# RainbowZL0/swin-unet-image-fusion

Measured on AMD Instinct MI355X. Metric: fused image-pairs/sec at 256x256, win=8, higher is better.
Workload: dtype bf16; 1 GPU; B=16/GPU 256x256 IR/visible pairs, win=8, 5-level Swin-UNet fusion forward (BASELINE configs[1]); global_batch=16, precision_mode=fast, residual_stream=fp32, hip_graph=True, steps_in_flight=3, kernel_schedule=throughput, collective=none, weights=random-init (numpy PCG64 recipe, seed 0)

## Files before the change

### swin_unet_image_fusion_amd/csrc/kernels_win96.hip

```cpp
#include "win_host.h"

#include <cstdlib>

namespace swf {
namespace {

using namespace wf;

template <int HID_>
struct G96 {
    static constexpr int C = 96, HID = HID_, HEADS = 8, D = 12, TC = 3, VT = 4, KS = 6;
    static constexpr int NT1 = HID / 32, KU = HID / 16;
    static_assert(HID % 32 == 0, "hidden tiles");
    static constexpr int F_QKV = 0;
    static constexpr int F_P = 144;
    static constexpr int F_W1 = 192;
    static constexpr int F_W2 = F_W1 + 12 * NT1;
    static constexpr int NFRAG = F_W2 + 6 * KU;
    static constexpr int V_LN1G = 0, V_LN1B = 48, V_LN2G = 96, V_LN2B = 144, V_B2 = 192, V_BQ = 240, V_BK = 304, V_B1 = 368;
    static constexpr int VHF = V_B1 + 16 * NT1, VSTREAM = 2 * VHF + 128;
    static constexpr size_t p_vec = size_t(NFRAG) * 1024;
    static constexpr size_t p_bias = (p_vec + size_t(VSTREAM) * 4 + 15) / 16 * 16;
    static constexpr size_t p_total = p_bias + size_t(2) * 2 * 16 * 64 * 4;
    static constexpr size_t l_k = 0, l_v = 32 * 1024, l_vec = 64 * 1024, l_total = l_vec + size_t(2) * VSTREAM * 4;
    static constexpr size_t l_vec8 = 96 * 1024, l_total8 = l_vec8 + size_t(2) * VSTREAM * 4;
    static constexpr size_t p_total16 = p_bias + size_t(15) * 16 * 64 * 4;
    static constexpr size_t l_k16 = 0, l_v16 = 64 * 1024, l_vec16 = 128 * 1024, l_total16 = l_vec16 + size_t(2) * VSTREAM * 4;
    static_assert(l_total16 <= 160 * 1024, "LDS");
};


__device__ __forceinline__ void layernorm96(const f32x16 (&x)[3], const float* vec, int goff, int boff, u32x4 (&xh)[6], u32x4 (&xl)[6]) {
    float s = 0.f;
#pragma unroll
    for (int T = 0; T < 3; ++T)
#pragma unroll
        for (int i = 0; i < 16; ++i) s += x[T][i];
    const float mean = sum_halves(s) * (1.0f / 96.0f);
    float q = 0.f;
#pragma unroll
    for (int T = 0; T < 3; ++T)
#pragma unroll
        for (int i = 0; i < 16; ++i) {
            const float d = x[T][i] - mean;
            q += d * d;
        }
    const float rstd = __builtin_amdgcn_rsqf(sum_halves(q) * (1.0f / 96.0f) + 1e-5f);
#pragma unroll
    for (int T = 0; T < 3; ++T) {
        float n[16];
#pragma unroll
        for (int a = 0; a < 4; ++a) {
            const float4 g = *reinterpret_cast<const float4*>(vec + goff + 16 * T + 4 * a);
            const float4 b = *reinterpret_cast<const float4*>(vec + boff + 16 * T + 4 * a);
            n[4 * a + 0] = (x[T][4 * a + 0] - mean) * rstd * g.x + b.x;
            n[4 * a + 1] = (x[T][4 * a + 1] - mean) * rstd * g.y + b.y;
            n[4 * a + 2] = (x[T][4 * a + 2] - mean) * rstd * g.z + b.z;
            n[4 * a + 3] = (x[T][4 * a + 3] - mean) * rstd * g.w + b.w;
        }
        split8(n, xh[2 * T], xl[2 * T]);
        split8(n + 8, xh[2 * T + 1], xl[2 * T + 1]);
    }
}

__device__ __forceinline__ void raw96(const f32x16 (&x)[3], u32x4 (&xh)[6], u32x4 (&xl)[6]) {
#pragma unroll
    for (int T = 0; T < 3; ++T) {
        float n[16];
#pragma unroll
        for (int i = 0; i < 16; ++i) n[i] = x[T][i];
        split8(n, xh[2 * T], xl[2 * T]);
        split8(n + 8, xh[2 * T + 1], xl[2 * T + 1]);
    }
}

template <int NH = 8>
__device__ __forceinline__ void attention96(const u32x4* ksrc, const u32x4* vsrc, const u32x4 (&qf)[NH / 2][2], const f32x16 (&bias)[2],
                                            bool half1, f32x16 (&o)[NH / 2]) {
    const f32x16 zero16 = {0.f, 0.f, 0.f, 0.f, 0.f, 0.f, 0.f, 0.f, 0.f, 0.f, 0.f, 0.f, 0.f, 0.f, 0.f, 0.f};
#pragma unroll
    for (int T = 0; T < NH / 2; ++T) o[T] = zero16;
#pragma unroll
    for (int h = 0; h < NH; ++h) {
        const int T = h >> 1, sp = h & 1;
        const u32x4 ka0 = ksrc[((0 * 4 + T) * 2 + sp) * 64], ka1 = ksrc[((1 * 4 + T) * 2 + sp) * 64];
        u32x4 qm = qf[T][sp];
        float mx;
        {
            f32x16 s0 = mfma_f16(ka0, qm, bias[0]);
            mx = max3f(s0[0], s0[1], s0[2]);
#pragma unroll
            for (int i = 3; i < 15; i += 2) mx = max3f(mx, s0[i], s0[i + 1]);
            mx = __builtin_fmaxf(mx, s0[15]);
        }
        {
            f32x16 s1 = mfma_f16(ka1, qm, bias[1]);
#pragma unroll
            for (int i = 0; i < 16; i += 2) mx = max3f(mx, s1[i], s1[i + 1]);
        }
        mx = max_halves(mx);
        {
            const f16 nm = (f16)(-mx);
            qm[2] |= half1 ? ((unsigned)__builtin_bit_cast(unsigned short, nm) << 16) : 0u;
        }
        f32x16 t;
#pragma unroll
        for (int kt = 0; kt < 2; ++kt) {
            f32x16 sc = mfma_f16(kt ? ka1 : ka0, qm, bias[kt]);
#pragma unroll
            for (int s2 = 0; s2 < 2; ++s2) {
                float p[8];
#pragma unroll
                for (int j = 0; j < 8; ++j) p[j] = __builtin_amdgcn_exp2f(sc[8 * s2 + j]);
                const u32x4 pf = pack8_f16(p);
                const u32x4 va = vsrc[(T * 4 + 2 * kt + s2) * 64];
                t = mfma_f16(va, pf, (kt == 0 && s2 == 0) ? zero16 : t);
                __builtin_amdgcn_sched_barrier(0);
            }
        }
#pragma unroll
        for (int j = 0; j < 8; ++j) o[T][8 * sp + j] = t[8 * sp + j];
        __builtin_amdgcn_sched_barrier(0);
    }
}

template <int HID, int WS, int MODE = WIN_BLOCK, bool RAW = false>
__global__ __launch_bounds__(256, 2) void window96_kernel(WinArgs args) {
    using G = G96<HID>;
    static_assert(WS == 7 || WS == 8, "window side");
    static_assert(!RAW || MODE != WIN_BLOCK, "RAW belongs to the half-block modes");
    constexpr bool ATT = MODE != WIN_MLP, MLP = MODE != WIN_ATTN;
    extern __shared__ __attribute__((aligned(16))) char smem96[];
    u32x4* kimg = reinterpret_cast<u32x4*>(smem96 + G::l_k);
    u32x4* vimg = reinterpret_cast<u32x4*>(smem96 + G::l_v);
    float* lvec = reinterpret_cast<float*>(smem96 + G::l_vec);

    const int tid = threadIdx.x, lane = tid & 63, wave = tid >> 6;
    const int ws = wave >> 1, qb = wave & 1, r = lane & 31, hf = lane >> 5;
    const int H = args.H, W = args.W, nwx = ATT ? W / WS : 1, nwy = ATT ? H / WS : 1, npi = nwx * nwy;
    const int nwin = ATT ? args.B * npi : (max(args.ntok[0], args.ntok[1]) + 63) / 64;
    const int sh = args.shift ? WS / 2 : 0;
    const int kvs = args.cross ? 1 - ws : ws;

    const __amdgpu_buffer_rsrc_t wrs = __builtin_amdgcn_make_buffer_rsrc(const_cast<char*>(uniform_ptr(args.packed[ws])), 0, (int)G::p_total, 0x00020000);
    const __amdgpu_buffer_rsrc_t krs = __builtin_amdgcn_make_buffer_rsrc(const_cast<char*>(uniform_ptr(args.packed[kvs])), 0, (int)G::p_total, 0x00020000);
    const int act_bytes = ATT ? args.B * H * W * 96 * 4 : args.ntok[ws] * 96 * 4;
    const __amdgpu_buffer_rsrc_t irs = __builtin_amdgcn_make_buffer_rsrc(const_cast<float*>(uniform_ptr(args.in[ws])), 0, act_bytes, 0x00020000);
    const __amdgpu_buffer_rsrc_t ors = __builtin_amdgcn_make_buffer_rsrc(uniform_ptr(args.out[ws]), 0, (MODE == WIN_BLOCK || args.out[ws]) ? act_bytes : 0, 0x00020000);
    const unsigned loff = (unsigned)lane * 16u;
    auto WF = [&](int f) { return __builtin_bit_cast(u32x4, __builtin_amdgcn_raw_buffer_load_b128(wrs, loff, f * 1024, 0)); };
    auto WK = [&](int f) { return __builtin_bit_cast(u32x4, __builtin_amdgcn_raw_buffer_load_b128(krs, loff, f * 1024, 0)); };
    const float* vec = lvec + ws * G::VSTREAM + hf * G::VHF;
    const float* veck = lvec + kvs * G::VSTREAM + hf * G::VHF;
    const float* vecv = lvec + kvs * G::VSTREAM + 2 * G::VHF;
    const bool half1 = hf != 0;
    const bool col_masked = half1 != (((r >> 2) & 1) != 0);
    const f32x16 zero16 = {0.f, 0.f, 0.f, 0.f, 0.f, 0.f, 0.f, 0.f, 0.f, 0.f, 0.f, 0.f, 0.f, 0.f, 0.f, 0.f};

    for (int win = blockIdx.x; win < nwin; win += gridDim.x) {
        SWF_WF_FENCE();
        const int b = win / npi, wrem = win - b * npi;
        const int wy = wrem / nwx, wx = wrem - wy * nwx;
        const int ty = 4 * qb + (r >> 3), tx = r & 7;
        int oy = wy * WS + ty + sh, ox = wx * WS + tx + sh;
        oy = oy >= H ? oy - H : oy;
        ox = ox >= W ? ox - W : ox;
        const unsigned tokoff = [&]() -> unsigned {
            if constexpr (ATT) {
                return (WS == 8 || (ty < WS && tx < WS)) ? (unsigned)((((b * H + oy) * W + ox) * 96 + 4 * hf) * 4) : 0x80000000u;
            } else {
                const int tok = 64 * win + 32 * qb + r;
                return tok < args.ntok[ws] ? (unsigned)((tok * 96 + 4 * hf) * 4) : 0x80000000u;
            }
        }();
        auto load_rows = [&](f32x16 (&x)[3]) {
#pragma unroll
            for (int a = 0; a < 12; ++a) {
                const f32x4 v = __builtin_bit_cast(f32x4, __builtin_amdgcn_raw_buffer_load_b128(irs, tokoff, 32 * a, 0));
                x[a >> 2][4 * (a & 3)] = v.x; x[a >> 2][4 * (a & 3) + 1] = v.y; x[a >> 2][4 * (a & 3) + 2] = v.z; x[a >> 2][4 * (a & 3) + 3] = v.w;
            }
        };

        f32x16 res[3];
        if constexpr (ATT) {
        u32x4 qf[4][2];
        {
            u32x4 wq[2][6];
            auto req = [&](int hp, u32x4 (&dst)[6]) {
                const int m = hp >> 3, f0 = G::F_QKV + ((hp >> 1) * 6 + 3 * (hp & 1)) * 2;
#pragma unroll
                for (int i = 0; i < 6; ++i) dst[i] = m == 0 ? WF(f0 + i) : WK(f0 + i);
            };
            req(0, wq[0]);
            u32x4 xh[6], xl[6];
            {
                f32x16 x[3];
                load_rows(x);
                if (win == (int)blockIdx.x) {
                    static_assert(G::VSTREAM % 4 == 0 && G::p_vec % 16 == 0, "vector sections move as 16-byte groups");
                    fill_vectors<G::VSTREAM / 4, 256>(lvec, args.packed[0] + G::p_vec, args.packed[1] + G::p_vec, tid);
                    __syncthreads();
                }
                if constexpr (RAW) raw96(x, xh, xl);
                else layernorm96(x, vec, G::V_LN1G, G::V_LN1B, xh, xl);
            }
            f32x16 acc = zero16;
#pragma unroll
            for (int hp = 0; hp < 24; ++hp) {
                const int m = hp >> 3, T = (hp >> 1) & 3, half = hp & 1;
                SWF_WF_FENCE();
                if (hp + 1 < 24) req(hp + 1, wq[(hp + 1) & 1]);
                SWF_WF_FENCE();
                const u32x4 (&w)[6] = wq[hp & 1];
                const bool skip = RAW && (m == 0 ? ws == 1 : ws == 0);
                if (skip && hp == 9 && win != (int)blockIdx.x) __syncthreads();
                if (half == 0) acc = zero16;
                if (!skip) {
#pragma unroll
                for (int s = 0; s < 3; ++s) {
                    const int ks = 3 * half + s;
                    acc = m < 2 ? mma3(w[2 * s], w[2 * s + 1], xh[ks], xl[ks], acc)
                                : mma3(xh[ks], xl[ks], w[2 * s], w[2 * s + 1], acc);
                }
                }
                if (half == 1 && !skip) {
                    float t[16];
                    if (m < 2) {
                        const float* bsrc = m == 0 ? vec + G::V_BQ : veck + G::V_BK;
#pragma unroll
                        for (int g = 0; g < 4; ++g) {
                            const float4 bb = *reinterpret_cast<const float4*>(bsrc + 16 * T + 4 * g);
                            t[4 * g] = acc[4 * g] + bb.x; t[4 * g + 1] = acc[4 * g + 1] + bb.y; t[4 * g + 2] = acc[4 * g + 2] + bb.z; t[4 * g + 3] = acc[4 * g + 3] + bb.w;
                        }
                        if (m == 0) {
                            qf[T][0] = pack8_f16(t);
                            qf[T][1] = pack8_f16(t + 8);
                        } else {
                            if (T == 0 && win != (int)blockIdx.x) __syncthreads();
                            u32x4* kdst = kimg + (((kvs * 2 + qb) * 4 + T) * 2) * 64 + lane;
                            kdst[0] = pack8_f16(t);
                            kdst[64] = pack8_f16(t + 8);
                        }
                    } else {
                        const float bv = vecv[32 * T + r];
#pragma unroll
                        for (int i = 0; i < 16; ++i) t[i] = acc[i] + bv;
                        u32x4* vdst = vimg + ((kvs * 4 + T) * 4 + 2 * qb) * 64 + lane;
                        vdst[0] = pack8_f16(t);
                        vdst[64] = pack8_f16(t + 8);
                    }
                }
            }
        }
        f32x16 bias[2];
        load_bias_tiles(wrs, loff, (int)G::p_bias, __builtin_amdgcn_readfirstlane(qb) * 2, bias);
        __syncthreads();
        if (RAW && ws == 1) continue;

        f32x16 o[4];
        {
            const bool rowv = args.shift && wy == nwy - 1, colv = args.shift && wx == nwx - 1;
            const u32x4* ksrc = kimg + (ws * 16) * 64 + lane;
            const u32x4* vsrc = vimg + (ws * 16) * 64 + lane;
            if (rowv || colv) {
                const float pen0 = ((rowv && qb == 1) || (colv && col_masked)) ? -INFINITY : 0.f;
                const float pen1 = ((rowv && qb == 0) || (colv && col_masked)) ? -INFINITY : 0.f;
#pragma unroll
                for (int i = 0; i < 16; ++i) { bias[0][i] += pen0; bias[1][i] += pen1; }
            }
            attention96(ksrc, vsrc, qf, bias, half1, o);
        }

        u32x4 wp[2][6];
        auto reqp = [&](int ks, u32x4 (&dst)[6]) {
#pragma unroll
            for (int To = 0; To < 3; ++To) { dst[2 * To] = WF(G::F_P + (To * 8 + ks) * 2); dst[2 * To + 1] = WF(G::F_P + (To * 8 + ks) * 2 + 1); }
        };
        SWF_WF_FENCE();
        if constexpr (RAW) { res[0] = zero16; res[1] = zero16; res[2] = zero16; }
        else load_rows(res);
        reqp(0, wp[0]);
        SWF_WF_FENCE();
        {
            u32x4 oh[8], ol[8];
#pragma unroll
            for (int h = 0; h < 8; ++h) {
                const int T = h >> 1, sp = h & 1;
                float lo_, den;
                halves(o[T][8 * sp + 4], lo_, den);
                const float inv = __builtin_amdgcn_rcpf(den);
                float t[8];
#pragma unroll
                for (int j = 0; j < 8; ++j) t[j] = o[T][8 * sp + j] * inv;
                split8(t, oh[h], ol[h]);
            }
#pragma unroll
            for (int ks = 0; ks < 8; ++ks) {
                SWF_WF_FENCE();
                if (ks + 1 < 8) reqp(ks + 1, wp[(ks + 1) & 1]);
                SWF_WF_FENCE();
                const u32x4 (&w)[6] = wp[ks & 1];
#pragma unroll
                for (int To = 0; To < 3; ++To) res[To] = mma3(w[2 * To], w[2 * To + 1], oh[ks], ol[ks], res[To]);
            }
        }

        } else {
            load_rows(res);
            if (win == (int)blockIdx.x) {
                fill_vectors<G::VSTREAM / 4, 256>(lvec, args.packed[0] + G::p_vec, args.packed[1] + G::p_vec, tid);
                __syncthreads();
            }
        }

        if constexpr (MLP) {
            u32x4 w1[12];
            auto req1 = [&](int tI) {
#pragma unroll
                for (int i = 0; i < 12; ++i) w1[i] = WF(G::F_W1 + tI * 12 + i);
            };
            req1(0);
            SWF_WF_FENCE();
            u32x4 xh[6], xl[6];
            if constexpr (RAW) { raw96(res, xh, xl); res[0] = zero16; res[1] = zero16; res[2] = zero16; }
            else layernorm96(res, vec, G::V_LN2G, G::V_LN2B, xh, xl);
#pragma unroll 1
            for (int tI = 0; tI < G::NT1; ++tI) {
                SWF_WF_FENCE();
                u32x4 w2[3][2][2];
#pragma unroll
                for (int To = 0; To < 3; ++To)
#pragma unroll
                    for (int s2 = 0; s2 < 2; ++s2) {
                        w2[To][s2][0] = WF(G::F_W2 + (To * G::KU + 2 * tI + s2) * 2);
                        w2[To][s2][1] = WF(G::F_W2 + (To * G::KU + 2 * tI + s2) * 2 + 1);
                    }
                SWF_WF_FENCE();
                f32x16 acc = zero16;
#pragma unroll
                for (int s = 0; s < 6; ++s) acc = mma3(w1[2 * s], w1[2 * s + 1], xh[s], xl[s], acc);
                SWF_WF_FENCE();
                if (tI + 1 < G::NT1) req1(tI + 1);
                SWF_WF_FENCE();
                float e[16];
                elu_tile(acc, vec + G::V_B1 + 16 * tI, e);
#pragma unroll
                for (int s2 = 0; s2 < 2; ++s2) {
                    u32x4 hh, hl;
                    split8(e + 8 * s2, hh, hl);
#pragma unroll
                    for (int To = 0; To < 3; ++To) res[To] = mma3(w2[To][s2][0], w2[To][s2][1], hh, hl, res[To]);
                }
            }
#pragma unroll
            for (int a = 0; a < 12; ++a) {
                const float4 b2 = *reinterpret_cast<const float4*>(vec + G::V_B2 + 4 * a);
                res[a >> 2][4 * (a & 3)] += b2.x; res[a >> 2][4 * (a & 3) + 1] += b2.y; res[a >> 2][4 * (a & 3) + 2] += b2.z; res[a >> 2][4 * (a & 3) + 3] += b2.w;
            }
        }

#pragma unroll
        for (int a = 0; a < 12; ++a) {
            const f32x4 v = {res[a >> 2][4 * (a & 3)], res[a >> 2][4 * (a & 3) + 1], res[a >> 2][4 * (a & 3) + 2], res[a >> 2][4 * (a & 3) + 3]};
            __builtin_amdgcn_raw_buffer_store_b128(__builtin_bit_cast(u32x4, v), ors, tokoff, 32 * a, 0);
        }
    }

    if (args.warm[0]) warm_next_block<256>(args, tid);
}


#ifdef W96_PROBE
__device__ unsigned long long w96_probe[16];
#define W96_STAMP(i) do { if (blockIdx.x == 0 && threadIdx.x == 0) w96_probe[i] = wall_clock64(); } while (0)
#else
#define W96_STAMP(i) do { } while (0)
#endif

template <int HID, int WS>
__global__ __launch_bounds__(512) void window96x8_kernel(WinArgs args) {
    using G = G96<HID>;
    static_assert(WS == 7 || WS == 8, "window side");
    static_assert(G::NT1 % 2 == 0, "hidden tiles split over the two feature halves");
    constexpr int NTH = G::NT1 / 2;
    extern __shared__ __attribute__((aligned(16))) char smem96[];
    u32x4* kimg = reinterpret_cast<u32x4*>(smem96 + G::l_k);
    u32x4* vimg = reinterpret_cast<u32x4*>(smem96 + G::l_v);
    f32x4* xch = reinterpret_cast<f32x4*>(smem96);
    float* lvec = reinterpret_cast<float*>(smem96 + G::l_vec8);

    const int tid = threadIdx.x, lane = tid & 63, wave = __builtin_amdgcn_readfirstlane(tid >> 6);
    const int ws = wave >> 2, qb = (wave >> 1) & 1, fh = wave & 1, r = lane & 31, hf = lane >> 5;
    const int H = args.H, W = args.W, nwx = W / WS, nwy = H / WS, npi = nwx * nwy;
    const int nwin = args.B * npi;
    const int sh = args.shift ? WS / 2 : 0;
    const int kvs = args.cross ? 1 - ws : ws;

    const __amdgpu_buffer_rsrc_t wrs = __builtin_amdgcn_make_buffer_rsrc(const_cast<char*>(uniform_ptr(args.packed[ws])), 0, (int)G::p_total, 0x00020000);
    const __amdgpu_buffer_rsrc_t krs = __builtin_amdgcn_make_buffer_rsrc(const_cast<char*>(uniform_ptr(args.packed[kvs])), 0, (int)G::p_total, 0x00020000);
    const int act_bytes = args.B * H * W * 96 * 4;
    const __amdgpu_buffer_rsrc_t irs = __builtin_amdgcn_make_buffer_rsrc(const_cast<float*>(uniform_ptr(args.in[ws])), 0, act_bytes, 0x00020000);
    const __amdgpu_buffer_rsrc_t ors = __builtin_amdgcn_make_buffer_rsrc(uniform_ptr(args.out[ws]), 0, act_bytes, 0x00020000);
    const unsigned loff = (unsigned)lane * 16u;
    auto WF = [&](int f) { return __builtin_bit_cast(u32x4, __builtin_amdgcn_raw_buffer_load_b128(wrs, loff, f * 1024, 0)); };
    auto WK = [&](int f) { return __builtin_bit_cast(u32x4, __builtin_amdgcn_raw_buffer_load_b128(krs, loff, f * 1024, 0)); };
    const float* vec = lvec + ws * G::VSTREAM + hf * G::VHF;
    const float* veck = lvec + kvs * G::VSTREAM + hf * G::VHF;
    const float* vecv = lvec + kvs * G::VSTREAM + 2 * G::VHF;
    const bool half1 = hf != 0;
    const bool col_masked = half1 != (((r >> 2) & 1) != 0);
    const f32x16 zero16 = {0.f, 0.f, 0.f, 0.f, 0.f, 0.f, 0.f, 0.f, 0.f, 0.f, 0.f, 0.f, 0.f, 0.f, 0.f, 0.f};
    auto put = [&](const f32x16 (&p)[3]) {
#pragma unroll
        for (int a = 0; a < 12; ++a)
            xch[(wave * 12 + a) * 64 + lane] = f32x4{p[a >> 2][4 * (a & 3)], p[a >> 2][4 * (a & 3) + 1], p[a >> 2][4 * (a & 3) + 2], p[a >> 2][4 * (a & 3) + 3]};
    };
    auto add_partner = [&](f32x16 (&p)[3]) {
#pragma unroll
        for (int a = 0; a < 12; ++a) {
            const f32x4 o = xch[((wave ^ 1) * 12 + a) * 64 + lane];
            p[a >> 2][4 * (a & 3)] += o[0]; p[a >> 2][4 * (a & 3) + 1] += o[1]; p[a >> 2][4 * (a & 3) + 2] += o[2]; p[a >> 2][4 * (a & 3) + 3] += o[3];
        }
    };

    W96_STAMP(0);
    for (int win = blockIdx.x; win < nwin; win += gridDim.x) {
        W96_STAMP(11 + (win != (int)blockIdx.x));
        SWF_WF_FENCE();
        const int b = win / npi, wrem = win - b * npi;
        const int wy = wrem / nwx, wx = wrem - wy * nwx;
        const int ty = 4 * qb + (r >> 3), tx = r & 7;
        int oy = wy * WS + ty + sh, ox = wx * WS + tx + sh;
        oy = oy >= H ? oy - H : oy;
        ox = ox >= W ? ox - W : ox;
        const unsigned tokoff = (WS == 8 || (ty < WS && tx < WS)) ? (unsigned)((((b * H + oy) * W + ox) * 96 + 4 * hf) * 4) : 0x80000000u;
        auto load_rows = [&](f32x16 (&x)[3]) {
#pragma unroll
            for (int a = 0; a < 12; ++a) {
                const f32x4 v = __builtin_bit_cast(f32x4, __builtin_amdgcn_raw_buffer_load_b128(irs, tokoff, 32 * a, 0));
                x[a >> 2][4 * (a & 3)] = v.x; x[a >> 2][4 * (a & 3) + 1] = v.y; x[a >> 2][4 * (a & 3) + 2] = v.z; x[a >> 2][4 * (a & 3) + 3] = v.w;
            }
        };

        u32x4 qf[2][2];
        {
            constexpr int PD = 4;
            u32x4 wq[PD][6];
            auto req = [&](int hp, u32x4 (&dst)[6]) {
                const int m = hp >> 2, f0 = G::F_QKV + ((m * 4 + ((hp >> 1) & 1)) * 6 + 3 * (hp & 1)) * 2 + fh * 24;
#pragma unroll
                for (int i = 0; i < 6; ++i) dst[i] = m == 0 ? WF(f0 + i) : WK(f0 + i);
            };
            req(0, wq[0]);
            u32x4 xh[6], xl[6];
            {
                f32x16 x[3];
                load_rows(x);
#pragma unroll
                for (int p = 1; p < PD - 1; ++p) req(p, wq[p]);
                if (win == (int)blockIdx.x) {
                    static_assert(G::VSTREAM % 4 == 0 && G::p_vec % 16 == 0, "vector sections move as 16-byte groups");
                    fill_vectors<G::VSTREAM / 4, 512>(lvec, args.packed[0] + G::p_vec, args.packed[1] + G::p_vec, tid);
                    __syncthreads();
                }
                layernorm96(x, vec, G::V_LN1G, G::V_LN1B, xh, xl);
            }
            W96_STAMP(1);
            f32x16 acc = zero16;
#pragma unroll
            for (int hp = 0; hp < 12; ++hp) {
                const int m = hp >> 2, Tl = (hp >> 1) & 1, half = hp & 1, T = 2 * fh + Tl;
                SWF_WF_FENCE();
                if (hp + PD - 1 < 12) req(hp + PD - 1, wq[(hp + PD - 1) % PD]);
                SWF_WF_FENCE();
                const u32x4 (&w)[6] = wq[hp % PD];
                if (half == 0) acc = zero16;
#pragma unroll
                for (int s = 0; s < 3; ++s) {
                    const int ks = 3 * half + s;
                    acc = m < 2 ? mma3(w[2 * s], w[2 * s + 1], xh[ks], xl[ks], acc)
                                : mma3(xh[ks], xl[ks], w[2 * s], w[2 * s + 1], acc);
                }
                if (half == 1) {
                    float t[16];
                    if (m < 2) {
                        const float* bsrc = m == 0 ? vec + G::V_BQ : veck + G::V_BK;
#pragma unroll
                        for (int g = 0; g < 4; ++g) {
                            const float4 bb = *reinterpret_cast<const float4*>(bsrc + 16 * T + 4 * g);
                            t[4 * g] = acc[4 * g] + bb.x; t[4 * g + 1] = acc[4 * g + 1] + bb.y; t[4 * g + 2] = acc[4 * g + 2] + bb.z; t[4 * g + 3] = acc[4 * g + 3] + bb.w;
                        }
                        if (m == 0) {
                            qf[Tl][0] = pack8_f16(t);
                            qf[Tl][1] = pack8_f16(t + 8);
                        } else {
                            if (Tl == 0 && win != (int)blockIdx.x) __syncthreads();
                            u32x4* kdst = kimg + (((kvs * 2 + qb) * 4 + T) * 2) * 64 + lane;
                            kdst[0] = pack8_f16(t);
                            kdst[64] = pack8_f16(t + 8);
                        }
                    } else {
                        const float bv = vecv[32 * T + r];
#pragma unroll
                        for (int i = 0; i < 16; ++i) t[i] = acc[i] + bv;
                        u32x4* vdst = vimg + ((kvs * 4 + T) * 4 + 2 * qb) * 64 + lane;
                        vdst[0] = pack8_f16(t);
                        vdst[64] = pack8_f16(t + 8);
                    }
                }
            }
        }
        W96_STAMP(2);
        f32x16 bias[2];
#pragma unroll
        for (int kt = 0; kt < 2; ++kt)
#pragma unroll
            for (int a = 0; a < 4; ++a) {
                const f32x4 v = __builtin_bit_cast(f32x4, __builtin_amdgcn_raw_buffer_load_b128(wrs, loff, (int)G::p_bias + ((qb * 2 + kt) * 4 + a) * 1024, 0));
                bias[kt][4 * a] = v.x; bias[kt][4 * a + 1] = v.y; bias[kt][4 * a + 2] = v.z; bias[kt][4 * a + 3] = v.w;
            }
        __syncthreads();
        W96_STAMP(3);

        f32x16 o[2];
        {
            const bool rowv = args.shift && wy == nwy - 1, colv = args.shift && wx == nwx - 1;
            const u32x4* ksrc = kimg + (ws * 16 + fh * 4) * 64 + lane;
            const u32x4* vsrc = vimg + (ws * 16 + fh * 8) * 64 + lane;
            if (rowv || colv) {
                const float pen0 = ((rowv && qb == 1) || (colv && col_masked)) ? -INFINITY : 0.f;
                const float pen1 = ((rowv && qb == 0) || (colv && col_masked)) ? -INFINITY : 0.f;
#pragma unroll
                for (int i = 0; i < 16; ++i) { bias[0][i] += pen0; bias[1][i] += pen1; }
            }
            attention96<4>(ksrc, vsrc, qf, bias, half1, o);
        }
        W96_STAMP(4);

        f32x16 res[3];
        {
            u32x4 wp[4][6];
#pragma unroll
            for (int ks = 0; ks < 4; ++ks)
#pragma unroll
                for (int To = 0; To < 3; ++To) {
                    wp[ks][2 * To] = WF(G::F_P + (To * 8 + ks) * 2 + fh * 8);
                    wp[ks][2 * To + 1] = WF(G::F_P + (To * 8 + ks) * 2 + 1 + fh * 8);
                }
            SWF_WF_FENCE();
            if (fh == 0) load_rows(res);
            else { res[0] = zero16; res[1] = zero16; res[2] = zero16; }
            SWF_WF_FENCE();
            u32x4 oh[4], ol[4];
#pragma unroll
            for (int h = 0; h < 4; ++h) {
                const int T = h >> 1, sp = h & 1;
                float lo_, den;
                halves(o[T][8 * sp + 4], lo_, den);
                const float inv = __builtin_amdgcn_rcpf(den);
                float t[8];
#pragma unroll
                for (int j = 0; j < 8; ++j) t[j] = o[T][8 * sp + j] * inv;
                split8(t, oh[h], ol[h]);
            }
#pragma unroll
            for (int ks = 0; ks < 4; ++ks)
#pragma unroll
                for (int To = 0; To < 3; ++To) res[To] = mma3(wp[ks][2 * To], wp[ks][2 * To + 1], oh[ks], ol[ks], res[To]);
        }
        W96_STAMP(5);
        __syncthreads();
        put(res);
        __syncthreads();
        add_partner(res);
        W96_STAMP(6);

        {
            u32x4 w1[12], w2[3][2][2];
            auto f1 = [&](int tI, int i) { return WF(G::F_W1 + tI * 12 + i + fh * (NTH * 12)); };
            auto f2 = [&](int tI, int To, int s2, int hl) { return WF(G::F_W2 + (To * G::KU + 2 * tI + s2) * 2 + hl + fh * (NTH * 4)); };
#pragma unroll
            for (int i = 0; i < 12; ++i) w1[i] = f1(0, i);
            SWF_WF_FENCE();
            u32x4 xh[6], xl[6];
            layernorm96(res, vec, G::V_LN2G, G::V_LN2B, xh, xl);
            if (fh != 0) { res[0] = zero16; res[1] = zero16; res[2] = zero16; }
            W96_STAMP(7);
#pragma unroll
            for (int s2 = 0; s2 < 2; ++s2)
#pragma unroll
                for (int To = 0; To < 3; ++To) { w2[To][s2][0] = f2(0, To, s2, 0); w2[To][s2][1] = f2(0, To, s2, 1); }
            SWF_WF_FENCE();
#pragma unroll 1
            for (int tI = 0; tI < NTH; ++tI) {
                const int tn = tI + 1 < NTH ? tI + 1 : tI;
                f32x16 acc = zero16;
#pragma unroll
                for (int s = 0; s < 6; ++s) {
                    acc = mma3(w1[2 * s], w1[2 * s + 1], xh[s], xl[s], acc);
                    SWF_WF_FENCE();
                    w1[2 * s] = f1(tn, 2 * s); w1[2 * s + 1] = f1(tn, 2 * s + 1);
                    SWF_WF_FENCE();
                }
                float e[16];
#pragma unroll
                for (int g = 0; g < 4; ++g) {
                    const float4 b1 = *reinterpret_cast<const float4*>(vec + G::V_B1 + 16 * (fh * NTH + tI) + 4 * g);
                    const float bb[4] = {b1.x, b1.y, b1.z, b1.w};
#pragma unroll
                    for (int j = 0; j < 4; ++j) {
                        const float u = acc[4 * g + j] + bb[j];
                        const float L = __builtin_fmaf(__builtin_amdgcn_exp2f(u), kLog2e, -kLog2e);
                        e[4 * g + j] = __builtin_amdgcn_fmed3f(u, L, 0.f);
                    }
                }
#pragma unroll
                for (int s2 = 0; s2 < 2; ++s2) {
                    u32x4 hh, hl;
                    split8(e + 8 * s2, hh, hl);
#pragma unroll
                    for (int To = 0; To < 3; ++To) {
                        res[To] = mma3(w2[To][s2][0], w2[To][s2][1], hh, hl, res[To]);
                        SWF_WF_FENCE();
                        w2[To][s2][0] = f2(tn, To, s2, 0); w2[To][s2][1] = f2(tn, To, s2, 1);
                        SWF_WF_FENCE();
                    }
                }
            }
        }
        W96_STAMP(8);
        __syncthreads();
        put(res);
        __syncthreads();
        add_partner(res);
#pragma unroll
        for (int a = 0; a < 12; ++a) {
            const float4 b2 = *reinterpret_cast<const float4*>(vec + G::V_B2 + 4 * a);
            res[a >> 2][4 * (a & 3)] += b2.x; res[a >> 2][4 * (a & 3) + 1] += b2.y; res[a >> 2][4 * (a & 3) + 2] += b2.z; res[a >> 2][4 * (a & 3) + 3] += b2.w;
        }

        W96_STAMP(9);
#pragma unroll
        for (int a = 0; a < 12; ++a) {
            if ((a >= 6) != (fh != 0)) continue;
            const f32x4 v = {res[a >> 2][4 * (a & 3)], res[a >> 2][4 * (a & 3) + 1], res[a >> 2][4 * (a & 3) + 2], res[a >> 2][4 * (a & 3) + 3]};
            __builtin_amdgcn_raw_buffer_store_b128(__builtin_bit_cast(u32x4, v), ors, tokoff, 32 * a, 0);
        }
    }

    W96_STAMP(10);
    if (args.warm[0]) {
        const int nsl = max(1, (int)gridDim.x / 8), sl = ((int)blockIdx.x / 8) % nsl;
        const int lines = (args.warm_bytes + 127) / 128;
        const int per = (lines + nsl - 1) / nsl, l0 = sl * per, l1 = min(lines, l0 + per);
        unsigned acc = 0;
        for (int s2 = 0; s2 < 2; ++s2)
            for (int l = l0 + tid; l < l1; l += 512) acc ^= *reinterpret_cast<const unsigned*>(args.warm[s2] + (size_t)l * 128);
        if (acc == 0x9e3779b9u && args.B < 0) args.out[0][0] = 0.f;
    }
}


template <int HID>
__global__ __launch_bounds__(256, 1) void window96w16_kernel(WinArgs args) {
    using G = G96<HID>;
    extern __shared__ __attribute__((aligned(16))) char smem96w[];
    u32x4* kimg = reinterpret_cast<u32x4*>(smem96w + G::l_k16);
    u32x4* vimg = reinterpret_cast<u32x4*>(smem96w + G::l_v16);
    float* lvec = reinterpret_cast<float*>(smem96w + G::l_vec16);

    const int tid = threadIdx.x, lane = tid & 63, wave = tid >> 6;
    const int ws = blockIdx.y, r = lane & 31, hf = lane >> 5;
    const int H = args.H, W = args.W, nwx = W / 16, nwy = H / 16, npi = nwx * nwy;
    const int nwin = args.B * npi;
    const int sh = args.shift ? 8 : 0;
    const int src = args.cross ? 1 - ws : ws;

    static_assert(G::VSTREAM % 4 == 0 && G::p_vec % 16 == 0, "vector sections move as 16-byte groups");
                    fill_vectors<G::VSTREAM / 4, 256>(lvec, args.packed[0] + G::p_vec, args.packed[1] + G::p_vec, tid);
    const __amdgpu_buffer_rsrc_t wrs = __builtin_amdgcn_make_buffer_rsrc(const_cast<char*>(args.packed[ws]), 0, (int)G::p_total16, 0x00020000);
    const int act_bytes = args.B * H * W * 96 * 4;
    const __amdgpu_buffer_rsrc_t irs = __builtin_amdgcn_make_buffer_rsrc(const_cast<float*>(args.in[ws]), 0, act_bytes, 0x00020000);
    const __amdgpu_buffer_rsrc_t srs = __builtin_amdgcn_make_buffer_rsrc(const_cast<float*>(args.in[src]), 0, act_bytes, 0x00020000);
    const __amdgpu_buffer_rsrc_t ors = __builtin_amdgcn_make_buffer_rsrc(args.out[ws], 0, act_bytes, 0x00020000);
    const unsigned loff = (unsigned)lane * 16u;
    auto WF = [&](int f) { return __builtin_bit_cast(u32x4, __builtin_amdgcn_raw_buffer_load_b128(wrs, loff, f * 1024, 0)); };
    const float* vec = lvec + ws * G::VSTREAM + hf * G::VHF;
    const float* vecs = lvec + src * G::VSTREAM + hf * G::VHF;
    const float* vecv = lvec + ws * G::VSTREAM + 2 * G::VHF;
    const bool half1 = hf != 0;
    const f32x16 zero16 = {0.f, 0.f, 0.f, 0.f, 0.f, 0.f, 0.f, 0.f, 0.f, 0.f, 0.f, 0.f, 0.f, 0.f, 0.f, 0.f};
    __syncthreads();

    for (int win = blockIdx.x; win < nwin; win += gridDim.x) {
        SWF_WF_FENCE();
        const int b = win / npi, wrem = win - b * npi;
        const int wy = wrem / nwx, wx = wrem - wy * nwx;
        auto tokoff_of = [&](int j) {
            int oy = wy * 16 + 2 * j + (r >> 4) + sh, ox = wx * 16 + (r & 15) + sh;
            oy = oy >= H ? oy - H : oy;
            ox = ox >= W ? ox - W : ox;
            return (unsigned)((((b * H + oy) * W + ox) * 96 + 4 * hf) * 4);
        };
        auto load_rows = [&](const __amdgpu_buffer_rsrc_t& rs, unsigned tokoff, f32x16 (&x)[3]) {
#pragma unroll
            for (int a = 0; a < 12; ++a) {
                const f32x4 v = __builtin_bit_cast(f32x4, __builtin_amdgcn_raw_buffer_load_b128(rs, tokoff, 32 * a, 0));
                x[a >> 2][4 * (a & 3)] = v.x; x[a >> 2][4 * (a & 3) + 1] = v.y; x[a >> 2][4 * (a & 3) + 2] = v.z; x[a >> 2][4 * (a & 3) + 3] = v.w;
            }
        };

        u32x4 qf[2][4][2];
#pragma unroll
        for (int jj = 0; jj < 2; ++jj)
#pragma unroll
            for (int T = 0; T < 4; ++T) { qf[jj][T][0] = u32x4{0u, 0u, 0u, 0u}; qf[jj][T][1] = u32x4{0u, 0u, 0u, 0u}; }
#pragma unroll 1
        for (int jj = 0; jj < 2; ++jj) {
            const int j = 2 * wave + jj;
            const unsigned tokoff = tokoff_of(j);
            u32x4 wq[2][6];
            auto req = [&](int hp, u32x4 (&dst)[6]) {
                const int f0 = G::F_QKV + ((hp >> 1) * 6 + 3 * (hp & 1)) * 2;
#pragma unroll
                for (int i = 0; i < 6; ++i) dst[i] = WF(f0 + i);
            };
            req(0, wq[0]);
            u32x4 xh[6], xl[6], kh[6], kl[6];
            {
                f32x16 x[3];
                load_rows(irs, tokoff, x);
                layernorm96(x, vec, G::V_LN1G, G::V_LN1B, xh, xl);
                if (args.cross) {
                    load_rows(srs, tokoff, x);
                    layernorm96(x, vecs, G::V_LN1G, G::V_LN1B, kh, kl);
                } else {
#pragma unroll
                    for (int s2 = 0; s2 < 6; ++s2) { kh[s2] = xh[s2]; kl[s2] = xl[s2]; }
                }
            }
#pragma unroll
            for (int T = 0; T < 4; ++T) { qf[0][T][0] = qf[1][T][0]; qf[0][T][1] = qf[1][T][1]; }
            f32x16 acc = zero16;
#pragma unroll
            for (int hp = 0; hp < 24; ++hp) {
                const int m = hp >> 3, T = (hp >> 1) & 3, half = hp & 1;
                SWF_WF_FENCE();
                if (hp + 1 < 24) req(hp + 1, wq[(hp + 1) & 1]);
                SWF_WF_FENCE();
                const u32x4 (&w)[6] = wq[hp & 1];
                if (half == 0) acc = zero16;
#pragma unroll
                for (int s2 = 0; s2 < 3; ++s2) {
                    const int ks = 3 * half + s2;
                    acc = m == 0 ? mma3(w[2 * s2], w[2 * s2 + 1], xh[ks], xl[ks], acc)
                        : m == 1 ? mma3(w[2 * s2], w[2 * s2 + 1], kh[ks], kl[ks], acc)
                                 : mma3(kh[ks], kl[ks], w[2 * s2], w[2 * s2 + 1], acc);
                }
                if (half == 1) {
                    float t[16];
                    if (m < 2) {
                        const float* bsrc = m == 0 ? vec + G::V_BQ : vec + G::V_BK;
#pragma unroll
                        for (int g = 0; g < 4; ++g) {
                            const float4 bb = *reinterpret_cast<const float4*>(bsrc + 16 * T + 4 * g);
                            t[4 * g] = acc[4 * g] + bb.x; t[4 * g + 1] = acc[4 * g + 1] + bb.y; t[4 * g + 2] = acc[4 * g + 2] + bb.z; t[4 * g + 3] = acc[4 * g + 3] + bb.w;
                        }
                        if (m == 0) {
                            qf[1][T][0] = pack8_f16(t);
                            qf[1][T][1] = pack8_f16(t + 8);
                        } else {
                            u32x4* kdst = kimg + ((j * 4 + T) * 2) * 64 + lane;
                            kdst[0] = pack8_f16(t);
                            kdst[64] = pack8_f16(t + 8);
                        }
                    } else {
                        const float bv = vecv[32 * T + r];
#pragma unroll
                        for (int i = 0; i < 16; ++i) t[i] = acc[i] + bv;
                        u32x4* vdst = vimg + (T * 16 + 2 * j) * 64 + lane;
                        vdst[0] = pack8_f16(t);
                        vdst[64] = pack8_f16(t + 8);
                    }
                }
            }
        }
        __syncthreads();

        const bool rowv = args.shift && wy == nwy - 1, colv = args.shift && wx == nwx - 1;
#pragma unroll 1
        for (int jj = 0; jj < 2; ++jj) {
            const int j = 2 * wave + jj;
            const unsigned tokoff = tokoff_of(j);
            f32x16 o[4] = {zero16, zero16, zero16, zero16};
            float mrun[8];
#pragma unroll
            for (int h = 0; h < 8; ++h) mrun[h] = -INFINITY;
#pragma unroll 1
            for (int c = 0; c < 4; ++c) {
                if (rowv && ((j < 4) != (c < 2))) continue;
                f32x16 bias[2];
                {
                    const int d0 = __builtin_amdgcn_readfirstlane(2 * c - j + 7);
                    load_bias_tiles(wrs, loff, (int)G::p_bias, d0, bias);
                    if (colv) col_seam16(bias, r);
                }
                const u32x4* kc = kimg + (2 * c) * 8 * 64 + lane;
#pragma unroll
                for (int h = 0; h < 8; ++h) {
                    const int T = h >> 1, sp = h & 1;
                    const u32x4 ka0 = kc[((0 * 4 + T) * 2 + sp) * 64], ka1 = kc[((1 * 4 + T) * 2 + sp) * 64];
                    u32x4 qm = qf[0][T][sp];
                    float mx;
                    {
                        f32x16 s0 = mfma_f16(ka0, qm, bias[0]);
                        mx = max3f(s0[0], s0[1], s0[2]);
#pragma unroll
                        for (int i = 3; i < 15; i += 2) mx = max3f(mx, s0[i], s0[i + 1]);
                        mx = __builtin_fmaxf(mx, s0[15]);
                    }
                    {
                        f32x16 s1 = mfma_f16(ka1, qm, bias[1]);
#pragma unroll
                        for (int i = 0; i < 16; i += 2) mx = max3f(mx, s1[i], s1[i + 1]);
                    }
                    mx = max_halves(mx);
                    const float mold = mrun[h];
                    const f16 nm = (f16)(-__builtin_fmaxf(mold, mx));
                    const float mnew = -(float)nm;
                    const float alpha = __builtin_amdgcn_exp2f(mold - mnew);
                    mrun[h] = mnew;
                    qm[2] |= half1 ? ((unsigned)__builtin_bit_cast(unsigned short, nm) << 16) : 0u;
                    f32x16 t;
#pragma unroll
                    for (int kt = 0; kt < 2; ++kt) {
                        f32x16 sc = mfma_f16(kt ? ka1 : ka0, qm, bias[kt]);
#pragma unroll
                        for (int s2 = 0; s2 < 2; ++s2) {
                            float pe[8];
#pragma unroll
                            for (int e = 0; e < 8; ++e) pe[e] = __builtin_amdgcn_exp2f(sc[8 * s2 + e]);
                            const u32x4 pf = pack8_f16(pe);
                            const u32x4 va = vimg[(T * 16 + 4 * c + 2 * kt + s2) * 64 + lane];
                            t = mfma_f16(va, pf, (kt == 0 && s2 == 0) ? zero16 : t);
                            __builtin_amdgcn_sched_barrier(0);
                        }
                    }
#pragma unroll
                    for (int e = 0; e < 8; ++e) o[T][8 * sp + e] = __builtin_fmaf(o[T][8 * sp + e], alpha, t[8 * sp + e]);
                    __builtin_amdgcn_sched_barrier(0);
                }
            }
#pragma unroll
            for (int T = 0; T < 4; ++T) { qf[0][T][0] = qf[1][T][0]; qf[0][T][1] = qf[1][T][1]; }

            f32x16 res[3];
            u32x4 wp[2][6];
            auto reqp = [&](int ks, u32x4 (&dst)[6]) {
#pragma unroll
                for (int To = 0; To < 3; ++To) { dst[2 * To] = WF(G::F_P + (To * 8 + ks) * 2); dst[2 * To + 1] = WF(G::F_P + (To * 8 + ks) * 2 + 1); }
            };
            SWF_WF_FENCE();
            load_rows(irs, tokoff, res);
            reqp(0, wp[0]);
            SWF_WF_FENCE();
            {
                u32x4 oh[8], ol[8];
#pragma unroll
                for (int h = 0; h < 8; ++h) {
                    const int T = h >> 1, sp = h & 1;
                    float lo_, den;
                    halves(o[T][8 * sp + 4], lo_, den);
                    const float inv = __builtin_amdgcn_rcpf(den);
                    float t[8];
#pragma unroll
                    for (int e = 0; e < 8; ++e) t[e] = o[T][8 * sp + e] * inv;
                    split8(t, oh[h], ol[h]);
                }
#pragma unroll
                for (int ks = 0; ks < 8; ++ks) {
                    SWF_WF_FENCE();
                    if (ks + 1 < 8) reqp(ks + 1, wp[(ks + 1) & 1]);
                    SWF_WF_FENCE();
                    const u32x4 (&w)[6] = wp[ks & 1];
#pragma unroll
                    for (int To = 0; To < 3; ++To) res[To] = mma3(w[2 * To], w[2 * To + 1], oh[ks], ol[ks], res[To]);
                }
            }
            {
                u32x4 xh[6], xl[6];
                layernorm96(res, vec, G::V_LN2G, G::V_LN2B, xh, xl);
                u32x4 w1[12];
                auto req1 = [&](int tI) {
#pragma unroll
                    for (int i = 0; i < 12; ++i) w1[i] = WF(G::F_W1 + tI * 12 + i);
                };
                req1(0);
#pragma unroll 1
                for (int tI = 0; tI < G::NT1; ++tI) {
                    SWF_WF_FENCE();
                    u32x4 w2[3][2][2];
#pragma unroll
                    for (int To = 0; To < 3; ++To)
#pragma unroll
                        for (int s2 = 0; s2 < 2; ++s2) {
                            w2[To][s2][0] = WF(G::F_W2 + (To * G::KU + 2 * tI + s2) * 2);
                            w2[To][s2][1] = WF(G::F_W2 + (To * G::KU + 2 * tI + s2) * 2 + 1);
                        }
                    SWF_WF_FENCE();
                    f32x16 acc = zero16;
#pragma unroll
                    for (int s2 = 0; s2 < 6; ++s2) acc = mma3(w1[2 * s2], w1[2 * s2 + 1], xh[s2], xl[s2], acc);
                    SWF_WF_FENCE();
                    if (tI + 1 < G::NT1) req1(tI + 1);
                    SWF_WF_FENCE();
                    float e[16];
                    elu_tile(acc, vec + G::V_B1 + 16 * tI, e);
#pragma unroll
                    for (int s2 = 0; s2 < 2; ++s2) {
                        u32x4 hh, hl;
                        split8(e + 8 * s2, hh, hl);
#pragma unroll
                        for (int To = 0; To < 3; ++To) res[To] = mma3(w2[To][s2][0], w2[To][s2][1], hh, hl, res[To]);
                    }
                }
#pragma unroll
                for (int a = 0; a < 12; ++a) {
                    const float4 b2 = *reinterpret_cast<const float4*>(vec + G::V_B2 + 4 * a);
                    res[a >> 2][4 * (a & 3)] += b2.x; res[a >> 2][4 * (a & 3) + 1] += b2.y; res[a >> 2][4 * (a & 3) + 2] += b2.z; res[a >> 2][4 * (a & 3) + 3] += b2.w;
                }
            }
#pragma unroll
            for (int a = 0; a < 12; ++a) {
                const f32x4 v = {res[a >> 2][4 * (a & 3)], res[a >> 2][4 * (a & 3) + 1], res[a >> 2][4 * (a & 3) + 2], res[a >> 2][4 * (a & 3) + 3]};
                __builtin_amdgcn_raw_buffer_store_b128(__builtin_bit_cast(u32x4, v), ors, tokoff, 32 * a, 0);
            }
        }
        __syncthreads();
    }
}

template <int HID>
__global__ __launch_bounds__(256) void pack96_kernel(WinPackArgs a) {
    using G = G96<HID>;
    const int st = blockIdx.y;
    const swf_block_stream_params& p = a.p[st];
    char* dst = a.dst[st];
    const int gtid = blockIdx.x * blockDim.x + threadIdx.x, gsz = gridDim.x * blockDim.x;
    const float qscale = kLog2e / sqrtf(12.0f);

    for (int idx = gtid; idx < G::NFRAG * 512; idx += gsz) {
        const int f = idx >> 9, lane = (idx >> 3) & 63, e = idx & 7, r = lane & 31, hf = lane >> 5;
        const int hl = f & 1;
        float val = 0.f;
        if (f < G::F_P) {
            const int g = f >> 1, s = g % 6, T = (g / 6) & 3, m = g / 24;
            const int k = kslot(s, hf, e), vch = 32 * T + r, head = vch >> 4, c = vch & 15;
            const swf_linear& l = m == 0 ? p.attn.q : m == 1 ? p.attn.k : p.attn.v;
            if (c < 12) {
                val = pack_wgt(l, (head * 12 + c) * 96 + k);
                if (m == 0) val *= qscale;
            }
        } else if (f < G::F_W1) {
            const int g = (f - G::F_P) >> 1, ks = g & 7, To = g >> 3;
            const int n = 32 * To + r, row = rho(e, hf);
            val = row < 12 ? pack_wgt(p.attn.proj, n * 96 + ks * 12 + row) : ((ks == 0 && row == 12) ? pack_bia(p.attn.proj, n) : 0.f);
        } else if (f < G::F_W2) {
            const int g = (f - G::F_W1) >> 1, s = g % 6, tI = g / 6;
            const int k = kslot(s, hf, e), hid = 32 * tI + r;
            val = pack_wgt(p.fc1, hid * 96 + k) * kLog2e;
        } else {
            const int g = (f - G::F_W2) >> 1, u = g % G::KU, To = g / G::KU;
            const int n = 32 * To + r, hid = kslot(u, hf, e);
            val = pack_wgt(p.fc2, n * HID + hid) * kLn2;
        }
        const bf16 hi = (bf16)val;
        reinterpret_cast<bf16*>(dst)[idx] = hl ? (bf16)(val - (float)hi) : hi;
    }
    float* vec = reinterpret_cast<float*>(dst + G::p_vec);
    for (int i = gtid; i < G::VSTREAM; i += gsz) {
        float v = 0.f;
        if (i < 2 * G::VHF) {
            const int hf = i / G::VHF, j = i % G::VHF;
            if (j < G::V_BQ) {
                const int which = j / 48, k = j % 48;
                const int c = 32 * (k >> 4) + rho(k & 15, hf);
                v = which == 0 ? (p.ln1.gamma ? p.ln1.gamma[c] : 1.f) : which == 1 ? (p.ln1.beta ? p.ln1.beta[c] : 0.f)
                  : which == 2 ? (p.ln2.gamma ? p.ln2.gamma[c] : 1.f) : which == 3 ? (p.ln2.beta ? p.ln2.beta[c] : 0.f) : pack_bia(p.fc2, c);
            } else if (j < G::V_B1) {
                const int isk = j >= G::V_BK, k = j - (isk ? G::V_BK : G::V_BQ), vch = 32 * (k >> 4) + rho(k & 15, hf);
                const int head = vch >> 4, c = vch & 15;
                if (c < 12) v = isk ? pack_bia(p.attn.k, head * 12 + c) : pack_bia(p.attn.q, head * 12 + c) * qscale;
                else if (isk && c == 13) v = 1.0f;
            } else {
                const int k = j - G::V_B1, hid = 32 * (k >> 4) + rho(k & 15, hf);
                v = pack_bia(p.fc1, hid) * kLog2e;
            }
        } else {
            const int vch = i - 2 * G::VHF, head = vch >> 4, c = vch & 15;
            v = c < 12 ? pack_bia(p.attn.v, head * 12 + c) : (c == 12 ? 1.0f : 0.f);
        }
        vec[i] = v;
    }
    if (p.attn.bias_table) pack_rel_bias<false>(reinterpret_cast<float*>(dst + G::p_bias), p.attn.bias_table, a.ws, gtid, gsz);
}

struct L96 {
    static constexpr int C = 96, D = 12, HID_WIDE = 384, HID_NARROW = 192, PACK_GRID = 128, WAVES = 2;
    static constexpr const char *name = "win96", *pack_name = "pack_win96";
    template <int HID> using G = G96<HID>;
    template <int HID>
    static void pack(dim3 grid, const WinPackArgs& a, hipStream_t stream) { hipLaunchKernelGGL((pack96_kernel<HID>), grid, dim3(256), 0, stream, a); }
    template <int HID, int WS, int MODE, bool RAW>
    static int launch(const swf_block_desc& d, const WinArgs& a, int grid, hipStream_t stream, int* route) {
        if constexpr (MODE == WIN_BLOCK) {
            static const bool no_x8 = [] { const char* e = debug_env("SWF_WIN96X8"); return e && e[0] == '0'; }();
            if (!no_x8 && d.schedule != SWF_SCHED_THROUGHPUT && (a.H / WS) * (a.W / WS) <= 16) {
                constexpr int lds8 = (int)G96<HID>::l_total8;
                SWF_TRY((raise_lds_limit<&window96x8_kernel<HID, WS>>(lds8, "window96x8")));
                trace_block(route, SWF_BLOCK_WIN_X8);
                hipLaunchKernelGGL((window96x8_kernel<HID, WS>), dim3(std::min(grid, num_cus())), dim3(512), lds8, stream, a);
                return check_launch("window96x8");
            }
        }
        constexpr int lds = (int)G96<HID>::l_total;
        SWF_TRY((raise_lds_limit<&window96_kernel<HID, WS, MODE, RAW>>(lds, MODE == WIN_BLOCK ? "window96" : "window96 half")));
        hipLaunchKernelGGL((window96_kernel<HID, WS, MODE, RAW>), dim3(grid), dim3(256), lds, stream, a);
        return check_launch(MODE == WIN_BLOCK ? "window96" : "window96 (half block)");
    }
    template <int HID>
    static int launch16(const WinArgs& a, int nwin, hipStream_t stream) {
        constexpr int lds = (int)G96<HID>::l_total16;
        SWF_TRY(raise_lds_limit<&window96w16_kernel<HID>>(lds, "window96w16"));
        hipLaunchKernelGGL((window96w16_kernel<HID>), dim3(std::min(nwin, (num_cus() + 1) / 2), 2), dim3(256), lds, stream, a);
        return check_launch("window96w16");
    }
};

}

const WinLevel& win96_level() {
    static const WinLevel level = win_level<L96>();
    return level;
}

}

#ifdef W96_PROBE
extern "C" int swf_w96_probe_read(unsigned long long* out) {
    return hipMemcpyFromSymbol(out, HIP_SYMBOL(swf::w96_probe), 16 * sizeof(unsigned long long)) == hipSuccess ? 0 : 1;
}
#endif
```

Before: 9197 pairs/s.

## Run two attention windows per 512-thread workgroup in throughput schedule

Adds a paired variant of the window96 kernel in which each 512-thread workgroup processes two windows, one per 256-thread half. Each half has its own K/V image in LDS, and the two halves share a single vector/bias section filled once. It is selected in throughput schedule when the number of window pairs fits within the CU count. This replaces the persistent-loop grid, cutting per-window vector refills and giving each CU one larger workgroup. The cost is that __syncthreads now couples both halves, and occupancy drops to one 512-thread block per CU.

```diff
diff --git a/swin_unet_image_fusion_amd/csrc/kernels_win96.hip b/swin_unet_image_fusion_amd/csrc/kernels_win96.hip
--- a/swin_unet_image_fusion_amd/csrc/kernels_win96.hip
+++ b/swin_unet_image_fusion_amd/csrc/kernels_win96.hip
@@ -23,6 +23,8 @@
     static constexpr size_t p_bias = (p_vec + size_t(VSTREAM) * 4 + 15) / 16 * 16;
     static constexpr size_t p_total = p_bias + size_t(2) * 2 * 16 * 64 * 4;
     static constexpr size_t l_k = 0, l_v = 32 * 1024, l_vec = 64 * 1024, l_total = l_vec + size_t(2) * VSTREAM * 4;
+    static constexpr size_t l_vecp = 128 * 1024, l_totalp = l_vecp + size_t(2) * VSTREAM * 4;
+    static_assert(l_totalp <= 160 * 1024, "LDS");
     static constexpr size_t l_vec8 = 96 * 1024, l_total8 = l_vec8 + size_t(2) * VSTREAM * 4;
     static constexpr size_t p_total16 = p_bias + size_t(15) * 16 * 64 * 4;
     static constexpr size_t l_k16 = 0, l_v16 = 64 * 1024, l_vec16 = 128 * 1024, l_total16 = l_vec16 + size_t(2) * VSTREAM * 4;
@@ -124,18 +126,21 @@
     }
 }
 
-template <int HID, int WS, int MODE = WIN_BLOCK, bool RAW = false>
-__global__ __launch_bounds__(256, 2) void window96_kernel(WinArgs args) {
+template <int HID, int WS, int MODE = WIN_BLOCK, bool RAW = false, bool PAIR = false>
+__global__ __launch_bounds__(PAIR ? 512 : 256, PAIR ? 1 : 2) void window96_kernel(WinArgs args) {
     using G = G96<HID>;
     static_assert(WS == 7 || WS == 8, "window side");
     static_assert(!RAW || MODE != WIN_BLOCK, "RAW belongs to the half-block modes");
+    static_assert(!PAIR || MODE == WIN_BLOCK, "the paired form runs whole blocks");
     constexpr bool ATT = MODE != WIN_MLP, MLP = MODE != WIN_ATTN;
     extern __shared__ __attribute__((aligned(16))) char smem96[];
-    u32x4* kimg = reinterpret_cast<u32x4*>(smem96 + G::l_k);
-    u32x4* vimg = reinterpret_cast<u32x4*>(smem96 + G::l_v);
-    float* lvec = reinterpret_cast<float*>(smem96 + G::l_vec);
-
-    const int tid = threadIdx.x, lane = tid & 63, wave = tid >> 6;
+    const int half = PAIR ? __builtin_amdgcn_readfirstlane((int)threadIdx.x >> 8) : 0;
+    char* simg = smem96 + (PAIR ? half * (int)G::l_vec : 0);
+    u32x4* kimg = reinterpret_cast<u32x4*>(simg + G::l_k);
+    u32x4* vimg = reinterpret_cast<u32x4*>(simg + G::l_v);
+    float* lvec = reinterpret_cast<float*>(smem96 + (PAIR ? G::l_vecp : G::l_vec));
+
+    const int tid = PAIR ? (int)threadIdx.x & 255 : (int)threadIdx.x, lane = tid & 63, wave = tid >> 6;
     const int ws = wave >> 1, qb = wave & 1, r = lane & 31, hf = lane >> 5;
     const int H = args.H, W = args.W, nwx = ATT ? W / WS : 1, nwy = ATT ? H / WS : 1, npi = nwx * nwy;
     const int nwin = ATT ? args.B * npi : (max(args.ntok[0], args.ntok[1]) + 63) / 64;
@@ -146,7 +151,8 @@
     const __amdgpu_buffer_rsrc_t krs = __builtin_amdgcn_make_buffer_rsrc(const_cast<char*>(uniform_ptr(args.packed[kvs])), 0, (int)G::p_total, 0x00020000);
     const int act_bytes = ATT ? args.B * H * W * 96 * 4 : args.ntok[ws] * 96 * 4;
     const __amdgpu_buffer_rsrc_t irs = __builtin_amdgcn_make_buffer_rsrc(const_cast<float*>(uniform_ptr(args.in[ws])), 0, act_bytes, 0x00020000);
-    const __amdgpu_buffer_rsrc_t ors = __builtin_amdgcn_make_buffer_rsrc(uniform_ptr(args.out[ws]), 0, (MODE == WIN_BLOCK || args.out[ws]) ? act_bytes : 0, 0x00020000);
+    const bool live = !PAIR || 2 * (int)blockIdx.x + half < nwin;
+    const __amdgpu_buffer_rsrc_t ors = __builtin_amdgcn_make_buffer_rsrc(uniform_ptr(args.out[ws]), 0, ((MODE == WIN_BLOCK || args.out[ws]) && live) ? act_bytes : 0, 0x00020000);
     const unsigned loff = (unsigned)lane * 16u;
     auto WF = [&](int f) { return __builtin_bit_cast(u32x4, __builtin_amdgcn_raw_buffer_load_b128(wrs, loff, f * 1024, 0)); };
     auto WK = [&](int f) { return __builtin_bit_cast(u32x4, __builtin_amdgcn_raw_buffer_load_b128(krs, loff, f * 1024, 0)); };
@@ -157,7 +163,8 @@
     const bool col_masked = half1 != (((r >> 2) & 1) != 0);
     const f32x16 zero16 = {0.f, 0.f, 0.f, 0.f, 0.f, 0.f, 0.f, 0.f, 0.f, 0.f, 0.f, 0.f, 0.f, 0.f, 0.f, 0.f};
 
-    for (int win = blockIdx.x; win < nwin; win += gridDim.x) {
+    for (int win = PAIR ? min(2 * (int)blockIdx.x + half, nwin - 1) : (int)blockIdx.x; PAIR || win < nwin; win += gridDim.x) {
+        auto first = [&] { return PAIR || win == (int)blockIdx.x; };
         SWF_WF_FENCE();
         const int b = win / npi, wrem = win - b * npi;
         const int wy = wrem / nwx, wx = wrem - wy * nwx;
@@ -196,9 +203,9 @@
             {
                 f32x16 x[3];
                 load_rows(x);
-                if (win == (int)blockIdx.x) {
+                if (first()) {
                     static_assert(G::VSTREAM % 4 == 0 && G::p_vec % 16 == 0, "vector sections move as 16-byte groups");
-                    fill_vectors<G::VSTREAM / 4, 256>(lvec, args.packed[0] + G::p_vec, args.packed[1] + G::p_vec, tid);
+                    fill_vectors<G::VSTREAM / 4, PAIR ? 512 : 256>(lvec, args.packed[0] + G::p_vec, args.packed[1] + G::p_vec, (int)threadIdx.x);
                     __syncthreads();
                 }
                 if constexpr (RAW) raw96(x, xh, xl);
@@ -213,7 +220,7 @@
                 SWF_WF_FENCE();
                 const u32x4 (&w)[6] = wq[hp & 1];
                 const bool skip = RAW && (m == 0 ? ws == 1 : ws == 0);
-                if (skip && hp == 9 && win != (int)blockIdx.x) __syncthreads();
+                if (skip && hp == 9 && !first()) __syncthreads();
                 if (half == 0) acc = zero16;
                 if (!skip) {
 #pragma unroll
@@ -236,7 +243,7 @@
                             qf[T][0] = pack8_f16(t);
                             qf[T][1] = pack8_f16(t + 8);
                         } else {
-                            if (T == 0 && win != (int)blockIdx.x) __syncthreads();
+                            if (T == 0 && !first()) __syncthreads();
                             u32x4* kdst = kimg + (((kvs * 2 + qb) * 4 + T) * 2) * 64 + lane;
                             kdst[0] = pack8_f16(t);
                             kdst[64] = pack8_f16(t + 8);
@@ -307,7 +314,7 @@
 
         } else {
             load_rows(res);
-            if (win == (int)blockIdx.x) {
+            if (first()) {
                 fill_vectors<G::VSTREAM / 4, 256>(lvec, args.packed[0] + G::p_vec, args.packed[1] + G::p_vec, tid);
                 __syncthreads();
             }
@@ -364,9 +371,17 @@
             const f32x4 v = {res[a >> 2][4 * (a & 3)], res[a >> 2][4 * (a & 3) + 1], res[a >> 2][4 * (a & 3) + 2], res[a >> 2][4 * (a & 3) + 3]};
             __builtin_amdgcn_raw_buffer_store_b128(__builtin_bit_cast(u32x4, v), ors, tokoff, 32 * a, 0);
         }
-    }
-
-    if (args.warm[0]) warm_next_block<256>(args, tid);
+        if constexpr (PAIR) break;
+    }
+
+    if (args.warm[0]) {
+        if constexpr (PAIR) {
+            if (2 * (int)blockIdx.x + 1 < nwin) warm_next_block<512>(args, (int)threadIdx.x);
+            else if (live) warm_next_block<256>(args, tid);
+        } else {
+            warm_next_block<256>(args, tid);
+        }
+    }
 }
 
 
@@ -1015,6 +1030,14 @@
     static int launch(const swf_block_desc& d, const WinArgs& a, int grid, hipStream_t stream, int* route) {
         if constexpr (MODE == WIN_BLOCK) {
             static const bool no_x8 = [] { const char* e = debug_env("SWF_WIN96X8"); return e && e[0] == '0'; }();
+            static const bool no_pair = [] { const char* e = debug_env("SWF_WIN96_PAIR"); return e && e[0] == '0'; }();
+            const int nwin = a.B * (a.H / WS) * (a.W / WS), pairs = (nwin + 1) / 2;
+            if (!no_pair && d.schedule == SWF_SCHED_THROUGHPUT && pairs <= num_cus()) {
+                constexpr int ldsp = (int)G96<HID>::l_totalp;
+                SWF_TRY((raise_lds_limit<&window96_kernel<HID, WS, WIN_BLOCK, false, true>>(ldsp, "window96 paired")));
+                hipLaunchKernelGGL((window96_kernel<HID, WS, WIN_BLOCK, false, true>), dim3(pairs), dim3(512), ldsp, stream, a);
+                return check_launch("window96 paired");
+            }
             if (!no_x8 && d.schedule != SWF_SCHED_THROUGHPUT && (a.H / WS) * (a.W / WS) <= 16) {
                 constexpr int lds8 = (int)G96<HID>::l_total8;
                 SWF_TRY((raise_lds_limit<&window96x8_kernel<HID, WS>>(lds8, "window96x8")));
```

New measurement: 9334 pairs/s (median of 6 runs). +1.5%, better.
